# Sinica-SLAM/speechbrain

Measured on AMD Instinct MI355X. Metric: audio-sec/sec Fbank→Conformer fwd (16kHz, B=32×15s) at 1/2/4/8 GPU, higher is better.
Workload: dtype bf16; 1 GPU; Fbank(80)→ConvFrontEnd(64,32)→Conformer 12L d=256 H=4 ffn=1024 k=31 encode, B=32×15s per GPU; global_batch=32, seq_len=376, parallelism=replicas1, hip_graph=True

## Files before the change

### speechbrain_amd/csrc/convmod.hip

```cpp
#include "mfma.h"

using namespace sbk;

namespace {

constexpr int CM_D = 256;
constexpr int CM_BM = 48;
constexpr int CM_KMAX = 31;
constexpr int CM_ROWS = 80;
constexpr int CM_MT1 = CM_ROWS / 16;
constexpr int CM_MT3 = CM_BM / 16;
constexpr int CM_NW = 16, CM_NT = CM_NW * 64;
constexpr int CM_S = CM_D + 16;
__device__ __forceinline__ constexpr int cm_sw(int row) { return ((row >> 2) & 1) << 3; }
static_assert(CM_NW % 8 == 0, "rows w + CM_NW * i share bit 2 with w (their swizzle is cm_sw(w))");

struct ConvModArgs {
  const float* x;
  float* out;
  int B, T, K, padL;
  const float *g0, *b0;
  float eps0;
  const bf16_t* w1;
  const float* b1;
  const float* wc;
  const float* bc;
  const float *g1, *b1n;
  float eps1;
  const bf16_t* w2;
  const float* b2;
  const uint8_t* kpm;
  const bf16_t* o;
  const bf16_t* wo;
  const float* bo;
  float inv_n, npad;
};

SBK_PROBE_BUFFER(g_cm_tl, 16, 8)
#define CM_TL(i) \
  SBK_PROBE(if (blockIdx.x == 100 && (threadIdx.x & 63) == 0) g_cm_tl[threadIdx.x >> 6][i] = __builtin_amdgcn_s_memtime();)

__device__ __forceinline__ void lds_barrier() {
  asm volatile("s_waitcnt lgkmcnt(0)" ::: "memory");
  __builtin_amdgcn_s_barrier();
  asm volatile("" ::: "memory");
}

__device__ __forceinline__ bf16x8 ld8g(const bf16_t* p) { return *reinterpret_cast<const bf16x8*>(p); }

#pragma clang diagnostic push
#pragma clang diagnostic ignored "-Winline-asm"
__device__ __forceinline__ void cm_dma(const bf16_t* src, bf16_t* lds) {
  const uint32_t la = __builtin_amdgcn_readfirstlane(
      (uint32_t)(uintptr_t)((__attribute__((address_space(3))) bf16_t*)lds));
  asm volatile("s_mov_b32 m0, %1\n\tglobal_load_lds_dwordx4 %0, off" ::"v"(src), "s"(la) : "memory", "m0");
}
#pragma clang diagnostic pop
__device__ __forceinline__ int cm_q(int q) { return ((((q ^ (q >> 1)) & 1) << 1) | (q >> 1)) & 3; }
__device__ __forceinline__ void cm_dma16(const bf16_t* src, bf16_t* dst, int lane) {
  const int r = lane >> 2, lc = (lane & 3) ^ cm_q((r >> 2) & 3);
  cm_dma(src + (long long)r * CM_D + 8 * lc, dst);
}
__device__ __forceinline__ bf16x8 cm_frag(const bf16_t* slot, int row, int g) {
  return *reinterpret_cast<const bf16x8*>(slot + row * 32 + 8 * (g ^ cm_q((row >> 2) & 3)));
}
__device__ __forceinline__ void cm_vmwait(int n) {
  if (n >= 2)
    asm volatile("s_waitcnt vmcnt(2)" ::: "memory");
  else if (n == 1)
    asm volatile("s_waitcnt vmcnt(1)" ::: "memory");
  else
    asm volatile("s_waitcnt vmcnt(0)" ::: "memory");
}
__device__ __forceinline__ f32x4 cm_gld4(const float* p) {
  f32x4 v;
  asm volatile("global_load_dwordx4 %0, %1, off" : "=v"(v) : "v"(p) : "memory");
  return v;
}
__device__ __forceinline__ void cm_tie(f32x4& v) { asm volatile("" : "+v"(v)); }
__device__ __forceinline__ int cm_gldu8(const uint8_t* p) {
  int v;
  asm volatile("global_load_ubyte %0, %1, off" : "=v"(v) : "v"(p) : "memory");
  return v;
}

template <bool PRE>
__global__ void __launch_bounds__(CM_NT) conv_module_kernel(ConvModArgs a) {
  extern __shared__ __attribute__((aligned(16))) unsigned char smem[];
  bf16_t* Us = reinterpret_cast<bf16_t*>(smem);
  bf16_t* Gs = Us + CM_ROWS * CM_S;
  float* Cv = reinterpret_cast<float*>(Gs + CM_ROWS * CM_S);

  const int tid = threadIdx.x, lane = tid & 63, w = tid >> 6;
  const int fr = lane & 15, g = lane >> 4, fk = 8 * g;
  const int fks = fk ^ cm_sw(fr);
  const int nblk = (a.T + CM_BM - 1) / CM_BM;
  const int tile = blockIdx.x;
  const int b = tile / nblk, t0 = (tile % nblk) * CM_BM;
  const int f0 = t0 - a.padL;
  const int nrows = CM_BM + a.K - 1;
  const long long ubase = (long long)b * a.T;
  CM_TL(0);
  constexpr int T1 = 2;
  constexpr int T3 = CM_D / 16 / CM_NW;
  constexpr int KSL = CM_D / 32, P1S = KSL * T1, SLOT = CM_NW * 16 * 32;
  bf16_t* p1slot[4] = {Gs, Gs + SLOT, reinterpret_cast<bf16_t*>(Cv), reinterpret_cast<bf16_t*>(Cv) + SLOT};
  bf16_t* const* p3slot = p1slot;
  static_assert(2 * SLOT * 2 <= CM_ROWS * CM_S * 2 && 2 * SLOT * 2 <= CM_BM * CM_D * 4, "ring slots fit");
  auto issue_p1 = [&](int q) __attribute__((always_inline)) {
    cm_dma16(a.w1 + (long long)(w * 32 + 16 * (q & 1)) * CM_D + 32 * (q >> 1), p1slot[q & 3] + w * 16 * 32, lane);
  };
  auto issue_p3 = [&](int ks) __attribute__((always_inline)) {
    cm_dma16(a.w2 + (long long)(w * 16) * CM_D + 32 * ks, p3slot[ks & 3] + w * 16 * 32, lane);
  };

  float4 xres[CM_MT3];
  if constexpr (PRE) {
    constexpr int OC = (CM_ROWS * (CM_D / 8) + CM_NT - 1) / CM_NT;
    uint4 ov[OC];
#pragma unroll
    for (int i = 0; i < OC; ++i) {
      const int c = min(tid + i * CM_NT, CM_ROWS * (CM_D / 8) - 1);
      const int r = c / (CM_D / 8), ch = c - r * (CM_D / 8);
      const int fc = min(max(f0 + r, 0), a.T - 1);
      ov[i] = *reinterpret_cast<const uint4*>(a.o + (ubase + fc) * CM_D + ch * 8);
    }
    float* lnscr = Cv + CM_NW * 32 * 32 / 2;
    static_assert(CM_NW * 32 * 32 / 2 + 2 * CM_ROWS * (CM_NW + 4) + 2 * CM_ROWS + 2 * CM_D <= CM_BM * CM_D,
                  "LN0 scratch fits beside the ring slot");
    float* gb0s = lnscr + 2 * CM_ROWS * (CM_NW + 4) + 2 * CM_ROWS;
    const float4 gbv = tid < CM_D / 2 ? *reinterpret_cast<const float4*>((tid < CM_D / 4 ? a.g0 : a.b0) +
                                                                         4 * (tid % (CM_D / 4)))
                                      : make_float4(0.f, 0.f, 0.f, 0.f);
    const int u0 = w * 16 + 4 * g;
    float4 xv[CM_MT1];
#pragma unroll
    for (int mt = 0; mt < CM_MT1; ++mt) {
      const int f = min(max(f0 + mt * 16 + fr, 0), a.T - 1);
      xv[mt] = *reinterpret_cast<const float4*>(a.x + (ubase + f) * CM_D + u0);
    }
    const float4 bo4 = a.bo ? *reinterpret_cast<const float4*>(a.bo + u0) : make_float4(0.f, 0.f, 0.f, 0.f);
    const bf16_t* wrowo = a.wo + (long long)(w * 16 + fr) * CM_D + fk;
    bf16x8 fwo[CM_D / 32];
#pragma unroll
    for (int kk = 0; kk < CM_D / 32; ++kk) fwo[kk] = ld8g(wrowo + kk * 32);
#pragma unroll
    for (int i = 0; i < OC; ++i) {
      const int c = tid + i * CM_NT;
      if (c < CM_ROWS * (CM_D / 8)) {
        const int r = c / (CM_D / 8), ch = c - r * (CM_D / 8), f = f0 + r;
        const bool live = r < nrows && f >= 0 && f < a.T;
        *reinterpret_cast<uint4*>(Gs + r * CM_S + ((ch * 8) ^ cm_sw(r))) = live ? ov[i] : uint4{0u, 0u, 0u, 0u};
      }
    }
    if (tid < CM_D / 2) *reinterpret_cast<float4*>(gb0s + 4 * tid) = gbv;
    CM_TL(6);
    lds_barrier();
    f32x4 acc[CM_MT1];
#pragma unroll
    for (int mt = 0; mt < CM_MT1; ++mt) acc[mt] = f32x4{0.f, 0.f, 0.f, 0.f};
#pragma unroll
    for (int kk = 0; kk < CM_D / 32; ++kk)
#pragma unroll
      for (int mt = 0; mt < CM_MT1; ++mt)
        acc[mt] = __builtin_amdgcn_mfma_f32_16x16x32_bf16(
            fwo[kk], *reinterpret_cast<const bf16x8*>(Gs + (mt * 16 + fr) * CM_S + kk * 32 + fks), acc[mt], 0, 0, 0);
    float xa[CM_MT1][4];
#pragma unroll
    for (int mt = 0; mt < CM_MT1; ++mt) {
      xa[mt][0] = xv[mt].x + (acc[mt][0] + bo4.x);
      xa[mt][1] = xv[mt].y + (acc[mt][1] + bo4.y);
      xa[mt][2] = xv[mt].z + (acc[mt][2] + bo4.z);
      xa[mt][3] = xv[mt].w + (acc[mt][3] + bo4.w);
    }
    {
      const int q = a.padL >> 4, rr = a.padL & 15;
      const int src = ((lane & 0x30) + ((fr + rr) & 15)) << 2;
      const bool hi = fr + rr >= 16;
#pragma unroll
      for (int mt = 0; mt < CM_MT3; ++mt) {
        float v[4];
#pragma unroll
        for (int e = 0; e < 4; ++e) {
          const float lo_v = q == 0 ? xa[mt][e] : xa[mt + 1][e];
          const float hi_v = q == 0 ? xa[mt + 1][e] : xa[mt + 2][e];
          const float lo = __int_as_float(__builtin_amdgcn_ds_bpermute(src, __float_as_int(lo_v)));
          const float hv = __int_as_float(__builtin_amdgcn_ds_bpermute(src, __float_as_int(hi_v)));
          v[e] = hi ? hv : lo;
        }
        xres[mt] = make_float4(v[0], v[1], v[2], v[3]);
      }
    }
    CM_TL(7);
    constexpr int RS = CM_NW + 4;
    float* red = lnscr;
    float mean[CM_MT1], rstd[CM_MT1];
#pragma unroll
    for (int mt = 0; mt < CM_MT1; ++mt) {
      const float ps = col4_sum((xa[mt][0] + xa[mt][1]) + (xa[mt][2] + xa[mt][3]));
      const float pq = col4_sum((xa[mt][0] * xa[mt][0] + xa[mt][1] * xa[mt][1]) +
                                (xa[mt][2] * xa[mt][2] + xa[mt][3] * xa[mt][3]));
      if (g == 0) {
        red[(mt * 16 + fr) * RS + w] = ps;
        red[CM_ROWS * RS + (mt * 16 + fr) * RS + w] = pq;
      }
    }
    lds_barrier();
    issue_p1(0);
    issue_p1(1);
    issue_p1(2);
    float* stat = red + 2 * CM_ROWS * RS;
    if (w < (CM_ROWS + 63) / 64 && w * 64 + lane < CM_ROWS) {
      const int row = w * 64 + lane;
      float t = 0.f, t2 = 0.f;
#pragma unroll
      for (int k4 = 0; k4 < CM_NW / 4; ++k4) {
        const float4 a4 = *reinterpret_cast<const float4*>(red + row * RS + 4 * k4);
        const float4 q4 = *reinterpret_cast<const float4*>(red + CM_ROWS * RS + row * RS + 4 * k4);
        t += a4.x;
        t += a4.y;
        t += a4.z;
        t += a4.w;
        t2 += q4.x;
        t2 += q4.y;
        t2 += q4.z;
        t2 += q4.w;
      }
      const float mu = t * a.inv_n;
      stat[row] = mu;
      stat[CM_ROWS + row] = 1.0f / sqrtf(fmaxf(t2 * a.inv_n - mu * mu, 0.f) + a.eps0);
    }
    lds_barrier();
    const float4 g04 = *reinterpret_cast<const float4*>(gb0s + u0);
    const float4 b04 = *reinterpret_cast<const float4*>(gb0s + CM_D + u0);
#pragma unroll
    for (int mt = 0; mt < CM_MT1; ++mt) {
      mean[mt] = stat[mt * 16 + fr];
      rstd[mt] = stat[CM_ROWS + mt * 16 + fr];
      const int r = mt * 16 + fr, f = f0 + r;
      const bool live = r < nrows && f >= 0 && f < a.T;
      uint2 pk = make_uint2(0u, 0u);
      if (live) {
        pk.x = pack_bf16x2((xa[mt][0] - mean[mt]) * rstd[mt] * g04.x + b04.x, (xa[mt][1] - mean[mt]) * rstd[mt] * g04.y + b04.y);
        pk.y = pack_bf16x2((xa[mt][2] - mean[mt]) * rstd[mt] * g04.z + b04.z, (xa[mt][3] - mean[mt]) * rstd[mt] * g04.w + b04.w);
      }
      *reinterpret_cast<uint2*>(Us + r * CM_S + (u0 ^ cm_sw(fr))) = pk;
    }
  } else {
  {
    constexpr int RPW = CM_ROWS / CM_NW;
    const float4 g04 = *reinterpret_cast<const float4*>(a.g0 + lane * 4);
    const float4 b04 = *reinterpret_cast<const float4*>(a.b0 + lane * 4);
    float4 xv[RPW];
#pragma unroll
    for (int i = 0; i < RPW; ++i) {
      const int r = w + i * CM_NW, f = min(max(f0 + r, 0), a.T - 1);
      xv[i] = *reinterpret_cast<const float4*>(a.x + (ubase + f) * CM_D + lane * 4);
    }
#pragma unroll
    for (int i = 0; i < RPW; ++i) {
      const int r = w + i * CM_NW, f = f0 + r;
      const bool live = r < nrows && f >= 0 && f < a.T;
      const float v[4] = {xv[i].x, xv[i].y, xv[i].z, xv[i].w};
      const float mean = wave_sum_v(v[0] + v[1] + v[2] + v[3]) * a.inv_n;
      float q = 0.f;
#pragma unroll
      for (int e = 0; e < 4; ++e) q += (v[e] - mean) * (v[e] - mean);
      const float rstd = 1.0f / sqrtf((wave_sum_v(q) - a.npad * mean * mean) * a.inv_n + a.eps0);
      uint2 pk = make_uint2(0u, 0u);
      if (live) {
        pk.x = pack_bf16x2((v[0] - mean) * rstd * g04.x + b04.x, (v[1] - mean) * rstd * g04.y + b04.y);
        pk.y = pack_bf16x2((v[2] - mean) * rstd * g04.z + b04.z, (v[3] - mean) * rstd * g04.w + b04.w);
      }
      *reinterpret_cast<uint2*>(Us + r * CM_S + ((lane * 4) ^ cm_sw(w))) = pk;
    }
  }
  }
  if constexpr (!PRE) {
    issue_p1(0);
    issue_p1(1);
    issue_p1(2);
  }
  lds_barrier();
  CM_TL(1);

  {
    f32x4 acc[T1][CM_MT1];
#pragma unroll
    for (int t = 0; t < T1; ++t)
#pragma unroll
      for (int mt = 0; mt < CM_MT1; ++mt) acc[t][mt] = f32x4{0.f, 0.f, 0.f, 0.f};
    bf16x8 fa[CM_MT1];
#pragma unroll
    for (int q = 0; q < P1S; ++q) {
      const int ks = q >> 1, t = q & 1;
      cm_vmwait(P1S - 1 - q < 2 ? P1S - 1 - q : 2);
      const bf16x8 fw = cm_frag(p1slot[q & 3], w * 16 + fr, g);
      if (t == 0) {
#pragma unroll
        for (int mt = 0; mt < CM_MT1; ++mt)
          fa[mt] = *reinterpret_cast<const bf16x8*>(Us + (mt * 16 + fr) * CM_S + ks * 32 + fks);
      }
      asm volatile("s_waitcnt lgkmcnt(0)" ::: "memory");
      if (q + 3 < P1S) issue_p1(q + 3);
#pragma unroll
      for (int mt = 0; mt < CM_MT1; ++mt)
        acc[t][mt] = __builtin_amdgcn_mfma_f32_16x16x32_bf16(fw, fa[mt], acc[t][mt], 0, 0, 0);
    }
    lds_barrier();
    {
      const int ch = w * 16 + 4 * g;
      const int pa = w * 32 + 4 * g, pg = pa + 16;
      const float4 ba = *reinterpret_cast<const float4*>(a.b1 + pa);
      const float4 bg = *reinterpret_cast<const float4*>(a.b1 + pg);
      const float bav[4] = {ba.x, ba.y, ba.z, ba.w}, bgv[4] = {bg.x, bg.y, bg.z, bg.w};
#pragma unroll
      for (int mt = 0; mt < CM_MT1; ++mt) {
        const int r = mt * 16 + fr, f = f0 + r;
        const bool live = r < nrows && f >= 0 && f < a.T;
        float o[4];
#pragma unroll
        for (int e = 0; e < 4; ++e) {
          const float va = acc[0][mt][e] + bav[e], vg = acc[1][mt][e] + bgv[e];
          const float sg = va * __builtin_amdgcn_rcpf(1.0f + __expf(-vg));
          o[e] = live ? sg : 0.f;
        }
        uint2 pk;
        pk.x = pack_bf16x2(o[0], o[1]);
        pk.y = pack_bf16x2(o[2], o[3]);
        *reinterpret_cast<uint2*>(Gs + r * CM_S + (ch ^ cm_sw(fr))) = pk;
      }
    }
  }
  lds_barrier();
  CM_TL(2);

  float4 xr[T3][CM_MT3];
  static_assert(T3 == 1, "phase 3: one 16-unit tile per wave (the units of phase -1)");
#pragma unroll
  for (int t = 0; t < T3; ++t)
#pragma unroll
    for (int mt = 0; mt < CM_MT3; ++mt) {
      const int f = min(t0 + mt * 16 + fr, a.T - 1);
      if constexpr (PRE)
        xr[t][mt] = xres[mt];
      else
        xr[t][mt] = *reinterpret_cast<const float4*>(a.x + (ubase + f) * CM_D + w * 16 * T3 + t * 16 + 4 * g);
    }

  {
    const int c = tid & (CM_D - 1), h = tid >> 8;
    constexpr int NF = CM_BM / (CM_NT / CM_D);
    constexpr int NP = (CM_KMAX + 1) / 2;
    float wk[2 * NP];
#pragma unroll
    for (int k = 0; k < 2 * NP; ++k) {
      const float v = a.wc[min(k, a.K - 1) * CM_D + c];
      wk[k] = k < a.K ? v : 0.f;
    }
    const float bias = a.bc ? a.bc[c] : 0.f;
    static_assert((CM_NT / CM_D) * NF + 2 * NP - 1 <= CM_ROWS, "every window row is staged");
    static_assert(NF % 2 == 0, "frame pairs");
    typedef __bf16 bf2 __attribute__((ext_vector_type(2)));
    bf2 tp[NP], ev[NF / 2 + NP - 1], od[NF / 2 + NP - 1];
#pragma unroll
    for (int j = 0; j < NP; ++j) {
      tp[j] = __builtin_bit_cast(bf2, pack_bf16x2(wk[2 * j], wk[2 * j + 1]));
      asm volatile("" : "+v"(tp[j]));
    }
    static_assert(NF % 4 == 0, "h * NF keeps bits 0-1 of the row");
    const int cx = c ^ cm_sw(h * NF);
    const unsigned short* Gu0 = reinterpret_cast<const unsigned short*>(Gs) + h * NF * CM_S + cx;
    const unsigned short* Gu1 = reinterpret_cast<const unsigned short*>(Gs) + h * NF * CM_S + (cx ^ 8);
    auto gu = [&](int k) __attribute__((always_inline)) { return (uint32_t)(cm_sw(k) ? Gu1 : Gu0)[k * CM_S]; };
    uint32_t g0 = gu(0);
#pragma unroll
    for (int r = 0; r < NF / 2 + NP - 1; ++r) {
      const uint32_t g1 = gu(2 * r + 1), g2 = gu(2 * r + 2);
      ev[r] = __builtin_bit_cast(bf2, g0 | (g1 << 16));
      od[r] = __builtin_bit_cast(bf2, g1 | (g2 << 16));
      g0 = g2;
    }
#pragma unroll
    for (int i = 0; i < NF; ++i) {
      float s = bias;
#pragma unroll
      for (int j = 0; j < NP; ++j) s = __builtin_amdgcn_fdot2_f32_bf16(tp[j], (i & 1) ? od[i / 2 + j] : ev[i / 2 + j], s, false);
      Cv[(h * NF + i) * CM_D + c] = s;
    }
  }
  lds_barrier();
  CM_TL(3);
  f32x4 bb2 = f32x4{0.f, 0.f, 0.f, 0.f};
  int km[CM_MT3] = {};
  {
    f32x4 g14 = cm_gld4(a.g1 + lane * 4), b14 = cm_gld4(a.b1n + lane * 4);
    if (a.b2) bb2 = cm_gld4(a.b2 + w * 16 * T3 + 4 * g);
    if (a.kpm) {
#pragma unroll
      for (int mt = 0; mt < CM_MT3; ++mt) km[mt] = cm_gldu8(a.kpm + ubase + min(t0 + mt * 16 + fr, a.T - 1));
    }
    issue_p3(0);
    issue_p3(1);
    asm volatile("s_waitcnt vmcnt(2)" ::: "memory");
    cm_tie(g14);
    cm_tie(b14);
    cm_tie(bb2);
#pragma unroll
    for (int mt = 0; mt < CM_MT3; ++mt) asm volatile("" : "+v"(km[mt]));
    const float gm[4] = {g14[0], g14[1], g14[2], g14[3]}, bt[4] = {b14[0], b14[1], b14[2], b14[3]};
    constexpr int FPW = CM_BM / CM_NW;
    float v[FPW][4], mean[FPW], rstd[FPW];
#pragma unroll
    for (int u = 0; u < FPW; ++u) {
      const float4 v4 = *reinterpret_cast<const float4*>(Cv + (w + u * CM_NW) * CM_D + lane * 4);
      v[u][0] = v4.x; v[u][1] = v4.y; v[u][2] = v4.z; v[u][3] = v4.w;
    }
#pragma unroll
    for (int u = 0; u < FPW; ++u) mean[u] = wave_sum_v((v[u][0] + v[u][1]) + (v[u][2] + v[u][3])) * a.inv_n;
#pragma unroll
    for (int u = 0; u < FPW; ++u) {
      float q = 0.f;
#pragma unroll
      for (int e = 0; e < 4; ++e) q += (v[u][e] - mean[u]) * (v[u][e] - mean[u]);
      rstd[u] = q;
    }
#pragma unroll
    for (int u = 0; u < FPW; ++u)
      rstd[u] = 1.0f / sqrtf((wave_sum_v(rstd[u]) - a.npad * mean[u] * mean[u]) * a.inv_n + a.eps1);
#pragma unroll
    for (int u = 0; u < FPW; ++u) {
#pragma unroll
      for (int e = 0; e < 4; ++e) {
        const float z = (v[u][e] - mean[u]) * rstd[u] * gm[e] + bt[e];
        v[u][e] = z * __builtin_amdgcn_rcpf(1.0f + __expf(-z));
      }
      uint2 pk;
      pk.x = pack_bf16x2(v[u][0], v[u][1]);
      pk.y = pack_bf16x2(v[u][2], v[u][3]);
      *reinterpret_cast<uint2*>(Us + (w + u * CM_NW) * CM_S + ((lane * 4) ^ cm_sw(w))) = pk;
    }
  }
  lds_barrier();
  CM_TL(4);

  {
    f32x4 acc[T3][CM_MT3];
#pragma unroll
    for (int t = 0; t < T3; ++t)
#pragma unroll
      for (int mt = 0; mt < CM_MT3; ++mt) acc[t][mt] = f32x4{0.f, 0.f, 0.f, 0.f};
    issue_p3(2);
#pragma unroll
    for (int ks = 0; ks < KSL; ++ks) {
      cm_vmwait(KSL - 1 - ks < 2 ? KSL - 1 - ks : 2);
      const bf16x8 fw = cm_frag(p3slot[ks & 3], w * 16 + fr, g);
      bf16x8 fa[CM_MT3];
#pragma unroll
      for (int mt = 0; mt < CM_MT3; ++mt)
        fa[mt] = *reinterpret_cast<const bf16x8*>(Us + (mt * 16 + fr) * CM_S + ks * 32 + fks);
      asm volatile("s_waitcnt lgkmcnt(0)" ::: "memory");
      if (ks + 3 < KSL) issue_p3(ks + 3);
#pragma unroll
      for (int mt = 0; mt < CM_MT3; ++mt)
        acc[0][mt] = __builtin_amdgcn_mfma_f32_16x16x32_bf16(fw, fa[mt], acc[0][mt], 0, 0, 0);
    }
#pragma unroll
    for (int t = 0; t < T3; ++t) {
      const int d = w * 16 * T3 + t * 16 + 4 * g;
      const f32x4 bb = bb2;
#pragma unroll
      for (int mt = 0; mt < CM_MT3; ++mt) {
        const int f = t0 + mt * 16 + fr;
        if (f >= a.T) continue;
        const bool m = km[mt] != 0;
        const float4 xv = xr[t][mt];
        float4 o;
        o.x = xv.x + (m ? 0.f : acc[t][mt][0] + bb[0]);
        o.y = xv.y + (m ? 0.f : acc[t][mt][1] + bb[1]);
        o.z = xv.z + (m ? 0.f : acc[t][mt][2] + bb[2]);
        o.w = xv.w + (m ? 0.f : acc[t][mt][3] + bb[3]);
        *reinterpret_cast<float4*>(a.out + (ubase + f) * CM_D + d) = o;
      }
    }
  }
  CM_TL(5);
}

constexpr size_t conv_module_lds() {
  return (size_t)2 * CM_ROWS * CM_S * sizeof(bf16_t) + (size_t)CM_BM * CM_D * sizeof(float);
}

}

SBK_PROBE_EXPORT(sbk_probe_cm_tl, g_cm_tl)

SBK_API int sbk_conv_module_supported(int D, int K) { return D == CM_D && K >= 1 && K <= CM_KMAX; }

SBK_API int sbk_conv_module_pre(const float* x, const void* o, const void* wo, const float* bo, float* out, int B,
                                int T, int D, int d_eff, const float* ln0_w, const float* ln0_b, float eps0, const void* w1p,
                                const float* b1p, const float* wc, const float* bc, int K, int causal,
                                const float* ln1_w, const float* ln1_b, float eps1, const void* w2, const float* b2,
                                const unsigned char* kpm, void* stream) {
  if (B <= 0 || T <= 0 || !sbk_conv_module_supported(D, K) || !x || !out || x == out || d_eff <= 0 || d_eff > D)
    return SBK_ERR_ARG;
  if (o && (causal ? K - 1 : (K - 1) / 2) > 31) return SBK_ERR_ARG;
  if (!ln0_w || !ln0_b || !w1p || !b1p || !wc || !ln1_w || !ln1_b || !w2) return SBK_ERR_ARG;
  const uintptr_t al = reinterpret_cast<uintptr_t>(x) | reinterpret_cast<uintptr_t>(out) |
                       reinterpret_cast<uintptr_t>(ln0_w) | reinterpret_cast<uintptr_t>(ln0_b) |
                       reinterpret_cast<uintptr_t>(w1p) | reinterpret_cast<uintptr_t>(b1p) |
                       reinterpret_cast<uintptr_t>(w2) | reinterpret_cast<uintptr_t>(b2);
  if (al & 15) return SBK_ERR_ARG;
  if ((o == nullptr) != (wo == nullptr) ||
      ((reinterpret_cast<uintptr_t>(o) | reinterpret_cast<uintptr_t>(wo) | reinterpret_cast<uintptr_t>(bo)) & 15))
    return SBK_ERR_ARG;
  ConvModArgs a;
  a.x = x; a.out = out; a.B = B; a.T = T; a.K = K; a.padL = causal ? K - 1 : (K - 1) / 2;
  a.g0 = ln0_w; a.b0 = ln0_b; a.eps0 = eps0;
  a.w1 = reinterpret_cast<const bf16_t*>(w1p); a.b1 = b1p;
  a.wc = wc; a.bc = bc;
  a.g1 = ln1_w; a.b1n = ln1_b; a.eps1 = eps1;
  a.w2 = reinterpret_cast<const bf16_t*>(w2); a.b2 = b2;
  a.kpm = reinterpret_cast<const uint8_t*>(kpm);
  a.o = reinterpret_cast<const bf16_t*>(o); a.wo = reinterpret_cast<const bf16_t*>(wo); a.bo = bo;
  a.inv_n = 1.0f / (float)d_eff; a.npad = (float)(D - d_eff);
  const long long grid = (long long)B * ((T + CM_BM - 1) / CM_BM);
  if (grid > 0x7fffffffLL) return SBK_ERR_ARG;
  constexpr size_t lds = conv_module_lds();
  static_assert(lds <= 160 * 1024, "LDS budget");
  for (const void* k : {reinterpret_cast<const void*>(&conv_module_kernel<false>),
                        reinterpret_cast<const void*>(&conv_module_kernel<true>)})
    if (hipError_t e = sbk::lds_optin(k, lds)) return (int)e;
  if (o)
    hipLaunchKernelGGL(conv_module_kernel<true>, dim3((unsigned)grid), dim3(CM_NT), lds, (hipStream_t)stream, a);
  else
    hipLaunchKernelGGL(conv_module_kernel<false>, dim3((unsigned)grid), dim3(CM_NT), lds, (hipStream_t)stream, a);
  SBK_CHECK_LAUNCH();
  return 0;
}

SBK_API int sbk_conv_module(const float* x, float* out, int B, int T, int D, int d_eff, const float* ln0_w,
                            const float* ln0_b,
                            float eps0, const void* w1p, const float* b1p, const float* wc, const float* bc, int K,
                            int causal, const float* ln1_w, const float* ln1_b, float eps1, const void* w2,
                            const float* b2, const unsigned char* kpm, void* stream) {
  return sbk_conv_module_pre(x, nullptr, nullptr, nullptr, out, B, T, D, d_eff, ln0_w, ln0_b, eps0, w1p, b1p, wc, bc, K,
                             causal, ln1_w, ln1_b, eps1, w2, b2, kpm, stream);
}
```

Baseline: 376,800 audio-sec/sec.

## Prefetch conv-module parameters at kernel start and stage them in LDS

Moves loads of the depthwise conv taps, conv bias, LN1 gamma/beta, pointwise biases, and key-padding mask to the start of the kernel. They are distributed across waves, then staged into a new LDS parameter region alongside the existing staging. Later phases read them from LDS instead of issuing global loads mid-kernel, which aims to take global latency off the critical path between phases. In exchange it adds LDS footprint, which may reduce occupancy, and keeps parameter registers live through the early phase. It also permits a null b1 bias.

Result: no change. 380,400 audio-sec/sec, median of 6 (+1.0%).

```diff
diff --git a/speechbrain_amd/csrc/convmod.hip b/speechbrain_amd/csrc/convmod.hip
--- a/speechbrain_amd/csrc/convmod.hip
+++ b/speechbrain_amd/csrc/convmod.hip
@@ -72,17 +72,28 @@
   else
     asm volatile("s_waitcnt vmcnt(0)" ::: "memory");
 }
-__device__ __forceinline__ f32x4 cm_gld4(const float* p) {
-  f32x4 v;
-  asm volatile("global_load_dwordx4 %0, %1, off" : "=v"(v) : "v"(p) : "memory");
-  return v;
-}
-__device__ __forceinline__ void cm_tie(f32x4& v) { asm volatile("" : "+v"(v)); }
-__device__ __forceinline__ int cm_gldu8(const uint8_t* p) {
-  int v;
-  asm volatile("global_load_ubyte %0, %1, off" : "=v"(v) : "v"(p) : "memory");
-  return v;
-}
+
+#define CM_GLOBAL __attribute__((address_space(1)))
+template <typename T>
+__device__ __forceinline__ const CM_GLOBAL T* cm_opaque(const T* p) {
+  asm volatile("" : "+s"(p));
+  return (const CM_GLOBAL T*)p;
+}
+__device__ __forceinline__ float4 cm_ld4(const CM_GLOBAL float* p) {
+  const f32x4 v = *(const CM_GLOBAL f32x4*)p;
+  return make_float4(v[0], v[1], v[2], v[3]);
+}
+
+constexpr int CM_NP = (CM_KMAX + 1) / 2;
+constexpr int CM_P_TP = 0;
+constexpr int CM_P_B1 = CM_P_TP + CM_NP * CM_D;
+constexpr int CM_P_BC = CM_P_B1 + 2 * CM_D;
+constexpr int CM_P_G1 = CM_P_BC + CM_D;
+constexpr int CM_P_B1N = CM_P_G1 + CM_D;
+constexpr int CM_P_B2 = CM_P_B1N + CM_D;
+constexpr int CM_P_KM = CM_P_B2 + CM_D;
+constexpr int CM_P_PAD = CM_P_KM + 64;
+constexpr int CM_P_FLOATS = CM_P_PAD + CM_D;
 
 template <bool PRE>
 __global__ void __launch_bounds__(CM_NT) conv_module_kernel(ConvModArgs a) {
@@ -114,6 +125,37 @@
     cm_dma16(a.w2 + (long long)(w * 16) * CM_D + 32 * ks, p3slot[ks & 3] + w * 16 * 32, lane);
   };
 
+  float* Ps = Cv + CM_BM * CM_D;
+  const int sc = tid & (CM_D - 1), sh = tid >> 8;
+  float stw[8], sbc;
+  float4 sv;
+  uint8_t skm;
+  const int ws = __builtin_amdgcn_readfirstlane(w);
+  const float* svp = ws < 2 ? (a.b1 ? a.b1 + ws * CM_D : a.g1) : ws == 3 ? a.b1n : ws == 4 && a.b2 ? a.b2 : a.g1;
+  const int svd = ws < 2 ? CM_P_B1 + ws * CM_D : ws == 2 ? CM_P_G1 : ws == 3 ? CM_P_B1N : ws == 4 ? CM_P_B2 : CM_P_PAD;
+  const bool svz = (ws < 2 && !a.b1) || (ws == 4 && !a.b2);
+  auto load_params = [&]() __attribute__((always_inline)) {
+#pragma unroll
+    for (int i = 0; i < 8; ++i) {
+      const int k = 8 * sh + i;
+      const float v = a.wc[min(k, a.K - 1) * CM_D + sc];
+      stw[i] = k < a.K ? v : 0.f;
+    }
+    sbc = cm_opaque(a.bc ? a.bc : a.g1)[sc];
+    sv = cm_ld4(cm_opaque(svp) + 4 * lane);
+    const uint8_t* kb = a.kpm ? a.kpm + ubase : reinterpret_cast<const uint8_t*>(a.g1);
+    skm = cm_opaque(kb)[a.kpm ? min(t0 + lane, a.T - 1) : lane];
+  };
+  load_params();
+  auto stage_params = [&]() __attribute__((always_inline)) {
+    uint32_t* tps = reinterpret_cast<uint32_t*>(Ps + CM_P_TP);
+#pragma unroll
+    for (int j = 0; j < 4; ++j) tps[(4 * sh + j) * CM_D + sc] = pack_bf16x2(stw[2 * j], stw[2 * j + 1]);
+    Ps[CM_P_BC + sc] = a.bc ? sbc : 0.f;
+    *reinterpret_cast<float4*>(Ps + svd + 4 * lane) = svz ? make_float4(0.f, 0.f, 0.f, 0.f) : sv;
+    reinterpret_cast<int*>(Ps + CM_P_KM)[lane] = a.kpm ? (int)skm : 0;
+  };
+
   float4 xres[CM_MT3];
   if constexpr (PRE) {
     constexpr int OC = (CM_ROWS * (CM_D / 8) + CM_NT - 1) / CM_NT;
@@ -139,7 +181,8 @@
       const int f = min(max(f0 + mt * 16 + fr, 0), a.T - 1);
       xv[mt] = *reinterpret_cast<const float4*>(a.x + (ubase + f) * CM_D + u0);
     }
-    const float4 bo4 = a.bo ? *reinterpret_cast<const float4*>(a.bo + u0) : make_float4(0.f, 0.f, 0.f, 0.f);
+    const float4 bov = cm_ld4(cm_opaque(a.bo ? a.bo : a.g0) + u0);
+    const float4 bo4 = a.bo ? bov : make_float4(0.f, 0.f, 0.f, 0.f);
     const bf16_t* wrowo = a.wo + (long long)(w * 16 + fr) * CM_D + fk;
     bf16x8 fwo[CM_D / 32];
 #pragma unroll
@@ -154,6 +197,7 @@
       }
     }
     if (tid < CM_D / 2) *reinterpret_cast<float4*>(gb0s + 4 * tid) = gbv;
+    stage_params();
     CM_TL(6);
     lds_barrier();
     f32x4 acc[CM_MT1];
@@ -257,6 +301,7 @@
       const int r = w + i * CM_NW, f = min(max(f0 + r, 0), a.T - 1);
       xv[i] = *reinterpret_cast<const float4*>(a.x + (ubase + f) * CM_D + lane * 4);
     }
+    stage_params();
 #pragma unroll
     for (int i = 0; i < RPW; ++i) {
       const int r = w + i * CM_NW, f = f0 + r;
@@ -311,8 +356,8 @@
     {
       const int ch = w * 16 + 4 * g;
       const int pa = w * 32 + 4 * g, pg = pa + 16;
-      const float4 ba = *reinterpret_cast<const float4*>(a.b1 + pa);
-      const float4 bg = *reinterpret_cast<const float4*>(a.b1 + pg);
+      const float4 ba = *reinterpret_cast<const float4*>(Ps + CM_P_B1 + pa);
+      const float4 bg = *reinterpret_cast<const float4*>(Ps + CM_P_B1 + pg);
       const float bav[4] = {ba.x, ba.y, ba.z, ba.w}, bgv[4] = {bg.x, bg.y, bg.z, bg.w};
 #pragma unroll
       for (int mt = 0; mt < CM_MT1; ++mt) {
@@ -351,23 +396,18 @@
   {
     const int c = tid & (CM_D - 1), h = tid >> 8;
     constexpr int NF = CM_BM / (CM_NT / CM_D);
-    constexpr int NP = (CM_KMAX + 1) / 2;
-    float wk[2 * NP];
-#pragma unroll
-    for (int k = 0; k < 2 * NP; ++k) {
-      const float v = a.wc[min(k, a.K - 1) * CM_D + c];
-      wk[k] = k < a.K ? v : 0.f;
-    }
-    const float bias = a.bc ? a.bc[c] : 0.f;
+    constexpr int NP = CM_NP;
     static_assert((CM_NT / CM_D) * NF + 2 * NP - 1 <= CM_ROWS, "every window row is staged");
     static_assert(NF % 2 == 0, "frame pairs");
     typedef __bf16 bf2 __attribute__((ext_vector_type(2)));
     bf2 tp[NP], ev[NF / 2 + NP - 1], od[NF / 2 + NP - 1];
+    const uint32_t* tps = reinterpret_cast<const uint32_t*>(Ps + CM_P_TP);
 #pragma unroll
     for (int j = 0; j < NP; ++j) {
-      tp[j] = __builtin_bit_cast(bf2, pack_bf16x2(wk[2 * j], wk[2 * j + 1]));
+      tp[j] = __builtin_bit_cast(bf2, tps[j * CM_D + c]);
       asm volatile("" : "+v"(tp[j]));
     }
+    const float bias = Ps[CM_P_BC + c];
     static_assert(NF % 4 == 0, "h * NF keeps bits 0-1 of the row");
     const int cx = c ^ cm_sw(h * NF);
     const unsigned short* Gu0 = reinterpret_cast<const unsigned short*>(Gs) + h * NF * CM_S + cx;
@@ -391,24 +431,12 @@
   }
   lds_barrier();
   CM_TL(3);
-  f32x4 bb2 = f32x4{0.f, 0.f, 0.f, 0.f};
-  int km[CM_MT3] = {};
   {
-    f32x4 g14 = cm_gld4(a.g1 + lane * 4), b14 = cm_gld4(a.b1n + lane * 4);
-    if (a.b2) bb2 = cm_gld4(a.b2 + w * 16 * T3 + 4 * g);
-    if (a.kpm) {
-#pragma unroll
-      for (int mt = 0; mt < CM_MT3; ++mt) km[mt] = cm_gldu8(a.kpm + ubase + min(t0 + mt * 16 + fr, a.T - 1));
-    }
     issue_p3(0);
     issue_p3(1);
-    asm volatile("s_waitcnt vmcnt(2)" ::: "memory");
-    cm_tie(g14);
-    cm_tie(b14);
-    cm_tie(bb2);
-#pragma unroll
-    for (int mt = 0; mt < CM_MT3; ++mt) asm volatile("" : "+v"(km[mt]));
-    const float gm[4] = {g14[0], g14[1], g14[2], g14[3]}, bt[4] = {b14[0], b14[1], b14[2], b14[3]};
+    const float4 g14 = *reinterpret_cast<const float4*>(Ps + CM_P_G1 + lane * 4);
+    const float4 b14 = *reinterpret_cast<const float4*>(Ps + CM_P_B1N + lane * 4);
+    const float gm[4] = {g14.x, g14.y, g14.z, g14.w}, bt[4] = {b14.x, b14.y, b14.z, b14.w};
     constexpr int FPW = CM_BM / CM_NW;
     float v[FPW][4], mean[FPW], rstd[FPW];
 #pragma unroll
@@ -468,7 +496,11 @@
 #pragma unroll
     for (int t = 0; t < T3; ++t) {
       const int d = w * 16 * T3 + t * 16 + 4 * g;
-      const f32x4 bb = bb2;
+      const float4 bb4 = *reinterpret_cast<const float4*>(Ps + CM_P_B2 + d);
+      const float bb[4] = {bb4.x, bb4.y, bb4.z, bb4.w};
+      int km[CM_MT3];
+#pragma unroll
+      for (int mt = 0; mt < CM_MT3; ++mt) km[mt] = reinterpret_cast<const int*>(Ps + CM_P_KM)[mt * 16 + fr];
 #pragma unroll
       for (int mt = 0; mt < CM_MT3; ++mt) {
         const int f = t0 + mt * 16 + fr;
@@ -488,7 +520,7 @@
 }
 
 constexpr size_t conv_module_lds() {
-  return (size_t)2 * CM_ROWS * CM_S * sizeof(bf16_t) + (size_t)CM_BM * CM_D * sizeof(float);
+  return (size_t)2 * CM_ROWS * CM_S * sizeof(bf16_t) + (size_t)(CM_BM * CM_D + CM_P_FLOATS) * sizeof(float);
 }
 
 }
@@ -505,7 +537,7 @@
   if (B <= 0 || T <= 0 || !sbk_conv_module_supported(D, K) || !x || !out || x == out || d_eff <= 0 || d_eff > D)
     return SBK_ERR_ARG;
   if (o && (causal ? K - 1 : (K - 1) / 2) > 31) return SBK_ERR_ARG;
-  if (!ln0_w || !ln0_b || !w1p || !b1p || !wc || !ln1_w || !ln1_b || !w2) return SBK_ERR_ARG;
+  if (!ln0_w || !ln0_b || !w1p || !wc || !ln1_w || !ln1_b || !w2) return SBK_ERR_ARG;
   const uintptr_t al = reinterpret_cast<uintptr_t>(x) | reinterpret_cast<uintptr_t>(out) |
                        reinterpret_cast<uintptr_t>(ln0_w) | reinterpret_cast<uintptr_t>(ln0_b) |
                        reinterpret_cast<uintptr_t>(w1p) | reinterpret_cast<uintptr_t>(b1p) |
```
